# chrished/DEMC.jl

Measured on AMD Instinct MI355X. Metric: chain-updates/sec (N x gens/s) + gens-to-Rhat<1.05, MvNormal d=5 N=1024, higher is better.
Workload: dtype f64

## Files before the change

### demc.jl_amd/csrc/demcz_capi.hip

```cpp
#include "../../include/demcz.h"
#include "demcz_kernels.h"
#include "demcz_kernels_acf.h"
#include "demcz_kernels_sel.h"
#include "demcz_select_host.h"
#include "demcz_kernels_ml.h"
#include "demcz_kernels_pc.h"
#include "demcz_kernels_lr.h"
#include "demcz_kernels_ps.h"
#include "demcz_kernels_ps2.h"
#include "demcz_kernels_ps2d.h"
#include "demcz_pw_dispatch.h"
#include "demcz_mlr_dispatch.h"
#include "demcz_program.h"

#include <rccl/rccl.h>

#include <algorithm>
#include <chrono>
#include <thread>
#include <cstdlib>
#include <deque>
#include <mutex>
#include <cmath>
#include <cstdio>
#include <cstring>
#include <string>
#include <unordered_map>
// ... 192 lines not shown
    bool external_append = false;
    double* dXprop = nullptr;
    double* dlogu = nullptr;
    bool proposal_pending = false;
    bool gen_open = false;
    double* hc_X = nullptr;
    double* hc_lp = nullptr;
    volatile unsigned int* hc_flag = nullptr;
    unsigned int* hc_count = nullptr;
    unsigned int hc_seq = 0;
    hipStream_t diag_stream = nullptr;
    hipEvent_t diag_ev = nullptr;
    hipEvent_t rhat_side_ev = nullptr;
    bool rhat_side_pending = false;
    double* d_spec_X = nullptr;
    double* d_spec_lp = nullptr;
    hipEvent_t spec_ev = nullptr;
    double* pinned_rhat = nullptr;
    unsigned int* pinned_err = nullptr;
    int64_t pinned_err_launches = -1;
    int64_t pinned_cap = 0;
    bool timing = false;
    std::vector<std::pair<hipEvent_t, hipEvent_t>> timed;
    std::vector<double> series_start_ms, series_dur_ms;
    int64_t timed_launches = 0;
    int64_t live_wg_cap = -1;
    SplitKind split_kind = SPLIT_NONE;
    int split_lanes = 0;
    int split_per_wg = 1;
    int32_t* d_slot_role = nullptr;
    double* d_rec[2] = {nullptr, nullptr};
    unsigned int* d_live_err = nullptr;
#ifdef DEMCZ_STAMPS
    unsigned long long* d_stamps = nullptr;
#endif
    bool arena = false, rec_in_arena = false, hist_joint = false;
    int64_t arena_gens = 0;
    double* arena_rec[2] = {nullptr, nullptr};
    double* arena_temp = nullptr;
    int64_t rec_cap = 0;
    int rec_cur = 0;
    bool host_paced = false;
    int wpw = 1;
    bool ps_dual = false;
    bool dual_now = false;
    bool lr_spec = false;
    bool no_live = false;
    bool live_claimed = false;
    unsigned int live_spin_limit = 0;
    int32_t live_fault_polls = 0;
    int64_t live_fault_g = 0;
    bool in_checked = false;
    struct RunCall { int64_t g_from, g_to; double gamma; bool tempered; std::vector<double> temperature; };
    std::vector<RunCall> live_log;
    double* d_safe_X = nullptr;
    double* d_safe_lp = nullptr;
    bool snap_pending = false;
    int64_t safe_M = 0, safe_M_app = 0, safe_g_done = 0;
    bool replaying = false;
    int32_t live_redos = 0;
// ... 260 lines not shown
static int32_t rec_scrub(demcz_handle* h)
{
    rec_invalidate(h);
    if (h->lanes != DEMCZ_LAYOUT_SPLIT || h->rec_cap <= 0 || getenv("DEMCZ_NO_SCRUB")) return DEMCZ_OK;
    for (int b = 0; b < 2; ++b) {
        if (!h->d_rec[b]) continue;
        const size_t per = h->rec_in_arena ? (size_t)(h->cfg.d + 2) : (size_t)((h->split_kind == SPLIT_MLB) ? 2 * h->S : (int64_t)h->cfg.d + 2);
        const size_t nd = (size_t)h->rec_cap * per * (size_t)h->cfg.N + REC_PAD;
        HIPCHK(h, hipMemsetAsync(h->d_rec[b], 0, nd * sizeof(double), h->stream));
    }
    return DEMCZ_OK;
}
static int32_t flush_exchanges(demcz_handle* h);
static void peer_detach(demcz_handle* h);
static void peer_no_dual(demcz_handle* h);
static int32_t peer_setup_ipc(demcz_handle* h);
static bool peer_capable(const demcz_handle* h);
static int32_t check_live_err(demcz_handle* h);
static int32_t live_verify(demcz_handle* h);
static int32_t group_verify(demcz_handle* h);
static int32_t live_failed(demcz_handle* h, bool& failed);
static void live_release(demcz_handle* h);
static int64_t live_span(demcz_handle* h);
static int32_t rec_reserve(demcz_handle* h, int64_t gens);
static int32_t check_hist_range(demcz_handle* h, int64_t g_from, int64_t g_to, const char* who);
static bool ps2_applicable(const demcz_handle* h, const WindowParams& P);

extern "C" int32_t demcz_abi_version(void) { return DEMCZ_ABI_VERSION; }

extern "C" const char* demcz_last_error(const demcz_handle* h)
{
    return h ? h->err.c_str() : g_create_error.c_str();
}

template <class T>
static hipError_t dev_alloc_copy(T** dst, const T* src, size_t n, hipStream_t s, int device)
{
    hipError_t e = dev_malloc(device, (void**)dst, std::max<size_t>(n, 1) * sizeof(T));
    if (e != hipSuccess) return e;
    if (n) e = hipMemcpyAsync(*dst, src, n * sizeof(T), hipMemcpyHostToDevice, s);
    return e;
}

static void free_all(demcz_handle* h)
{
    bool drained = !h->comm_dead;
// ... 263 lines not shown
            h->lanes = L;
        } else if (cfg->lanes_per_chain == 0 && L > 1 && cfg->N * L <= 262144) {
            h->lanes = L;
        }
    }
    if (h->lanes == DEMCZ_LAYOUT_SPLIT && h->split_kind == SPLIT_ML && cfg->target_kind == DEMCZ_TARGET_LINREG_SSE && !getenv("DEMCZ_NO_LR_SPEC")) {
        int cus = 0;
        if (hipDeviceGetAttribute(&cus, hipDeviceAttributeMultiprocessorCount, cfg->device_id) != hipSuccess) cus = 0;
        if ((cfg->N + LR8_CHAINS - 1) / LR8_CHAINS <= (int64_t)cus && lr8s_dynamic_lds<10>(cfg->nobs) <= ML_MAX_DYNAMIC_LDS) {
            h->lr_spec = true;
            h->split_per_wg = LR8_CHAINS;
        }
    }
    h->cfg.block_offsets = nullptr; h->cfg.block_indices = nullptr; h->cfg.eps_scale = nullptr;
    h->cfg.mu = nullptr; h->cfg.W = nullptr; h->cfg.design = nullptr; h->cfg.yobs = nullptr; h->cfg.stream = nullptr;
    if (cfg->target_kind == DEMCZ_TARGET_PROGRAM) h->cfg.nobs = 0;

    const int64_t N = cfg->N;
    const int64_t N_for_arena = cfg->N;
    h->ZS = (d <= 1) ? 2 : (d <= 2) ? 2 : (d <= 4) ? 4 : ((d + 7) / 8) * 8;
    {
        size_t zbytes = (size_t)cfg->Mcap * h->ZS * sizeof(double);
        if (h->lanes == DEMCZ_LAYOUT_SPLIT && h->split_kind == SPLIT_WAVE && d <= 5 && !h->prog_wave && !getenv("DEMCZ_NO_PS2")) {
            const int64_t per_gen = (int64_t)(d + 2) * N_for_arena * (int64_t)sizeof(double);
            int64_t ag = std::max<int64_t>(cfg->K, std::min<int64_t>((int64_t)((h->ps_dual ? 128ll : 64ll) << 20) / per_gen, 1 << 20));
            if (cfg->Gcap > 0) ag = std::min<int64_t>(ag, std::max<int64_t>(cfg->Gcap, 1024));
            ag = std::max<int64_t>(ag, (int64_t)cfg->K * 4);
            const size_t zb = (zbytes + 255) & ~(size_t)255;
            const size_t rb = (((size_t)ag * (size_t)(d + 2) * (size_t)N_for_arena + REC_PAD) * sizeof(double) + 255) & ~(size_t)255;
            const size_t tb = (((size_t)ag + 64) * sizeof(double) + 255) & ~(size_t)255;
            if (zb + 2 * rb + tb < 0xF0000000ull) {
                h->arena = true;
                h->arena_gens = ag;
                CRCHK(g_dev_pool.acquire((void**)&h->dZ, zb + 2 * rb + tb, cfg->device_id));
                h->dZ_bytes = zb + 2 * rb + tb;
                unsigned char* base = reinterpret_cast<unsigned char*>(h->dZ);
                h->arena_rec[0] = reinterpret_cast<double*>(base + zb);
                h->arena_rec[1] = reinterpret_cast<double*>(base + zb + rb);
                h->arena_temp = reinterpret_cast<double*>(base + zb + 2 * rb);
                CRCHK(hipMemsetAsync(base + zb, 0, 2 * rb + tb, h->stream));
            }
        }
        if (!h->arena) { CRCHK(g_dev_pool.acquire((void**)&h->dZ, zbytes, cfg->device_id)); h->dZ_bytes = zbytes; }
        if (h->ps_dual && !h->arena) { h->ps_dual = false; h->split_per_wg = PS_CHAINS; h->live_wg_cap = -1; }
        h->pooled_dev = true;
    }
    CRCHK(dev_malloc(h->cfg.device_id, (void**)&h->d_live_err, 4 * sizeof(unsigned int)));
    CRCHK(hipMemsetAsync(h->d_live_err, 0, 4 * sizeof(unsigned int), h->stream));
    CRCHK(dev_malloc(h->cfg.device_id, (void**)&h->dX, (size_t)N * d * sizeof(double)));
    CRCHK(dev_malloc(h->cfg.device_id, (void**)&h->dlp, (size_t)N * sizeof(double)));
    if (cfg->Gcap > 0) {
        const size_t skew = getenv("DEMCZ_DEBUG_HIST_SKEW") ? ((size_t)atol(getenv("DEMCZ_DEBUG_HIST_SKEW")) & ~(size_t)7) : 0;
        CRCHK(g_dev_pool.acquire((void**)&h->dchain_alloc, (size_t)N * (d + 1) * cfg->Gcap * sizeof(double) + skew, cfg->device_id));
        h->dchain = h->dchain_alloc + skew / sizeof(double);
        h->dlogobj = h->dchain + (size_t)N * d * cfg->Gcap;
        h->hist_joint = true;
// ... 1252 lines not shown
    std::lock_guard<std::mutex> lk(g_live_mutex);
    const int dev = h->cfg.device_id;
    if (dev >= 0 && dev < 64) g_live_used[dev] = std::max<int64_t>(0, g_live_used[dev] - h->live_share);
    h->live_share = 0;
    h->live_claimed = false;
}

static void peer_no_dual(demcz_handle* h)
{
    if (!h->ps_dual) return;
    live_release(h);
    h->ps_dual = false;
    h->dual_now = false;
    h->split_per_wg = PS_CHAINS;
    h->live_wg_cap = -1;
    rec_invalidate(h);
}

static bool peer_capable(const demcz_handle* h)
{
    return h->lanes == DEMCZ_LAYOUT_SPLIT && h->split_kind != SPLIT_PC8 && h->split_kind != SPLIT_NONE;
}

static int64_t live_span(demcz_handle* h)
{
    if (h->lanes != DEMCZ_LAYOUT_SPLIT || (h->comm && h->peer_mode != 2) || h->lag > 0 || h->external_append || h->no_live) return 0;
    if (h->peer_mode != 0 && !peer_capable(h)) return 0;
    if (h->peer_mode == 1 && (!h->group || h->group->failed || h->group->dead)) return 0;
    static const bool disabled = (getenv("DEMCZ_NO_LIVE") != nullptr);
    if (disabled) return 0;
    const int per_wg = h->split_per_wg;
    if ((h->cfg.N + per_wg - 1) / per_wg > live_wg_capacity(h)) return 0;
    if (!live_claim(h)) return 0;
    const int64_t per_gen = rec_fields(h) * h->cfg.N * (int64_t)sizeof(double);
    static const int64_t env_mib = getenv("DEMCZ_REC_MIB") ? atol(getenv("DEMCZ_REC_MIB")) : 0;
    const int64_t mib = env_mib > 0 ? env_mib : (h->arena ? (h->ps_dual ? 128 : 64) : (h->split_kind == SPLIT_MLB) ? 128 : 1024);
    const int64_t span = (int64_t)(mib << 20) / per_gen;
    return std::max<int64_t>(h->cfg.K, std::min<int64_t>(span, 1 << 20));
}

static int32_t stream_history(demcz_handle* h, int64_t g_from, int64_t g_to)
{
    if (!h->hs_on || h->cfg.Gcap <= 0 || g_to < g_from) return DEMCZ_OK;
    const int64_t N = h->cfg.N, s0 = g_from - h->g0 - 1, G = g_to - g_from + 1;
    const int d = h->cfg.d;
    if (s0 < 0 || s0 + G > h->cfg.Gcap) return DEMCZ_OK;
    hipEvent_t ev = h->after_launch_ev;
    if (!ev) {
        if (!h->diag_ev) HIPCHK(h, hipEventCreateWithFlags(&h->diag_ev, hipEventDisableTiming));
        HIPCHK(h, hipEventRecord(h->diag_ev, h->stream));
        h->after_launch_ev = ev = h->diag_ev;
    }
    HIPCHK(h, hipStreamWaitEvent(h->hs_stream, ev, 0));
    HIPCHK(h, hipMemcpyAsync(h->hs_chain + (size_t)N * d * s0, h->dchain + (size_t)N * d * s0, (size_t)N * d * G * sizeof(double), hipMemcpyDeviceToHost, h->hs_stream));
    HIPCHK(h, hipMemcpyAsync(h->hs_logobj + (size_t)N * s0, h->dlogobj + (size_t)N * s0, (size_t)N * G * sizeof(double), hipMemcpyDeviceToHost, h->hs_stream));
    return DEMCZ_OK;
}

extern "C" int32_t demcz_history_stream(demcz_handle* h, int32_t enabled)
// ... 210 lines not shown
        if (h->ps_dual) {
            const int64_t tb0 = next_boundary - g + 1, rest = g_to - g + 1;
            const bool temp_ok = !temperature || temp_in_arena;
            const bool hist_ok = !hist || (double)h->cfg.N * (h->cfg.d + 1) * (double)h->cfg.Gcap * 8.0 < 4293918720.0;
            const bool reg = K % PS2_R == 0 && tb0 % PS2_R == 0 && rest >= PS2_R && temp_ok && hist_ok && h->arena && h->rec_in_arena;
            if (reg) {
                h->dual_now = true;
                if (live_max > 0) live_max = std::max<int64_t>((std::min(live_max, rest) / PS2_R) * PS2_R, PS2_R);
                else w_end = g + ((w_end - g + 1) / PS2_R) * PS2_R - 1;
            } else {
                live_max = 0;
            }
        }
        if (live_max > 0) {
            int64_t n = std::min(live_max, g_to - g + 1);
            const auto& dc = h->rec_desc[h->rec_cur];
            const int64_t rows_v = h->cfg.N * (peer ? shards : 1);
            const int32_t boff = (int32_t)(K - (next_boundary - g + 1));
            const bool ready = dc.valid && dc.g_first == g + h->rng_offset && dc.M == h->M && dc.rows == rows_v && dc.boff == boff;
            if (ready && dc.ngen >= K) {
                if (dc.ngen < n) n = std::max<int64_t>((dc.ngen / K) * K, K);
            } else {
                const int64_t per_gen = rec_fields(h) * h->cfg.N * (int64_t)sizeof(double);
                const int64_t cold = std::max<int64_t>(K, ((int64_t)((h->ps_dual ? 128ll : 64ll) << 20) / per_gen / K) * K);
                n = std::min(n, cold);
            }
            if (h->dual_now) n = std::max<int64_t>((n / PS2_R) * PS2_R, PS2_R);
            w_end = g + n - 1;
        }
        int32_t rc = admit_pending(h, g);
        if (rc) return rc;
        const int64_t nbound = w_end / K - (g - 1) / K;
        P.M = h->M;
        P.M_append = h->M_app;
        P.g_first = g + h->rng_offset;
        P.ngen = (int32_t)(w_end - g + 1);
        P.to_boundary = (int32_t)(next_boundary - g + 1);
        P.slot_first = hist ? (g - h->g0 - 1) : 0;
        P.temperature = temperature ? (temp_in_arena ? h->arena_temp : h->dtemp) + (g - g_from) : nullptr;
        P.do_append = (nbound > 0 && kernel_appends) ? 1 : 0;
        P.snap = nullptr;
        if (nbound > 0 && rccl_exchange && E > 0) {
            if (h->batch_cnt == 0) {
                if (h->buf_xseq[h->batch_buf] > h->xseq_waited) HIPCHK(h, hipStreamWaitEvent(h->stream, h->buf_done[h->batch_buf], 0));
                h->batch_base = h->M_app;
            }
            P.snap = h->d_send[h->batch_buf] + (size_t)h->batch_cnt * h->cfg.N * h->cfg.d;
        }
        if (h->lanes == DEMCZ_LAYOUT_SPLIT) {
            const int64_t ng = w_end + 1;
            const int64_t nb1 = ((ng - 1) / K + 1) * (int64_t)K;
            int64_t nend = nb1;
            if (E > 0 && !h->external_append) nend = ((nend / K + E - 1) / E) * E * (int64_t)K;
            int64_t nM = h->M, nn = nend - ng + 1;
            const int64_t rows_n = h->cfg.N * shards;
            if (live_max > 0) nn = std::min(live_max, (w_end < g_to) ? g_to - w_end : G);
            if (h->external_append) nn = 0;
            else if (E == 0) nM = h->M_app + nbound * rows_n;
            else for (const auto& pe : h->pending) if (pe.visible_from <= ng) nM = pe.M_after;
            const int64_t vis_rows = (E == 0) ? rows_n : 0;
            const int32_t nboff = (int32_t)(K - (nb1 - ng + 1));
            rc = pc_prepare(h, P, vis_rows, ng + h->rng_offset, nn, nM, vis_rows, nboff);
            if (rc) return rc;
        }
        static const bool force_live = getenv("DEMCZ_FORCE_LIVE_KERNEL") != nullptr;
        const bool live = live_max > 0 && (((w_end - 1) / K - (g - 1) / K) > 0 || peer || force_live);
        P.live_err = h->d_live_err;
        P.live_spin_limit = h->live_spin_limit ? (int32_t)h->live_spin_limit : LIVE_SPIN_LIMIT;
        if (h->live_fault_polls > 0 && g >= h->live_fault_g) P.live_spin_limit = h->live_fault_polls;
        if (h->live_fault_polls < 0 && live && g >= h->live_fault_g)
            HIPCHK(h, hipMemsetAsync(h->d_live_err, 0x01, sizeof(unsigned int), h->stream));
        P.acc_out = h->d_acc ? h->d_acc + (size_t)h->acc_next * (size_t)h->acc_waves * 2 : nullptr;
        if (h->ps_dual && P.acc_out)
            HIPCHK(h, hipMemsetAsync(P.acc_out, 0, (size_t)h->acc_waves * 2 * sizeof(unsigned int), h->stream));
        if (live) h->err_clean = false;
        rc = launch_window(h, P, live);
        h->after_launch_ev = nullptr;
        if (rc) return rc;
        if (h->d_acc) {
// ... 11 lines not shown
            } else {
                for (int64_t j = (g - 1) / K + 1; j <= w_end / K; ++j) {
                    const int64_t J = ((j + E - 1) / E) * E;
                    h->M_app += rows;
                    if (h->batch_J != J) {
                        h->pending.push_back({(J + E) * (int64_t)K + 1, h->M_app, nullptr});
                        h->batch_J = J;
                    } else {
                        h->pending.back().M_after = h->M_app;
                    }
                    if (rccl_exchange) {
                        ++h->batch_cnt;
                        if (j == J) { rc = exchange_batch(h); if (rc) return rc; }
                    }
                }
            }
        }
        g = w_end + 1;
    }
    if (timed) {
        HIPCHK(h, hipEventRecord(tev.b, h->stream));
        h->after_launch_ev = tev.b;
        h->timed.emplace_back(tev.a, tev.b);
        tev.a = tev.b = nullptr;
        h->timed_launches += timed_launches;
    }
    if (rccl_exchange && E > 0) {
        int32_t rc = exchange_batch(h);
        if (rc) return rc;
    }
    h->g_done = g_to;
    return DEMCZ_OK;
}

extern "C" int32_t demcz_synchronize(demcz_handle* h)
{
    if (!h) return DEMCZ_ERR_INVALID_ARGUMENT;
    DEADCHK(h);
    HIPCHK(h, hipSetDevice(h->cfg.device_id));
    SYNCCHK(h, h->stream);
    if (h->comm_stream) SYNCCHK(h, h->comm_stream);
    if (h->prod_stream) SYNCCHK(h, h->prod_stream);
    return live_verify(h);
}

static int32_t check_hist_range(demcz_handle* h, int64_t g_from, int64_t g_to, const char* who)
// ... 91 lines not shown
        rc = ensure_scratch(h, 1);
        if (rc) return rc;
        static_assert(sizeof(long long) == sizeof(double), "scratch reuse");
        hipLaunchKernelGGL(sum_counts_kernel, dim3(1), dim3(256), 0, h->stream, (const unsigned int*)h->d_acc, h->acc_waves,
                           (int)h->acc_log[first].slot, last - first + 1, (int)h->acc_slots, skip, (long long*)h->d_scratch);
        HIPCHK(h, hipGetLastError());
        long long v = 0;
        HIPCHK(h, hipMemcpyAsync(&v, h->d_scratch, sizeof(v), hipMemcpyDeviceToHost, h->stream));
        SYNCCHK(h, h->stream);
        *total = (int64_t)v;
        if (from_ballots) *from_ballots = 1;
        return DEMCZ_OK;
    }
    std::vector<int64_t> ch((size_t)(g_to - g_from + 1));
    rc = demcz_get_changed(h, g_from, g_to, ch.data());
    if (rc) return rc;
    int64_t t = 0;
    for (int64_t v : ch) t += v;
    *total = t;
    if (from_ballots) *from_ballots = 0;
    return DEMCZ_OK;
}

struct RhatPlan { int64_t N, w, s0, n, nd, need; int d, nchunk; double *S1, *S2, *mean_j, *s2_j, *sums; };

static int rhat_chunks(int64_t n) { return (int)std::min<int64_t>(std::max<int64_t>(1, n / 32), 32); }
static int64_t rhat_need(int64_t nd, int d, int nchunk) { return 2 * (2 * nchunk * nd) + 2 * (2 * nd) + 4 * d; }

static int32_t rhat_plan(demcz_handle* h, int64_t g_from, int64_t g_to, RhatPlan& r, const char* who = "demcz_rhat")
{
    int32_t rc = check_hist_range(h, g_from, g_to, who);
    if (rc) return rc;
    r.N = h->cfg.N; r.w = g_to - g_from + 1; r.s0 = g_from - h->g0 - 1; r.d = h->cfg.d;
    r.n = r.w / 2;
    if (r.n < 2) return fail(h, DEMCZ_ERR_INVALID_ARGUMENT, std::string(who) + ": window needs at least 4 generations");
    r.nchunk = rhat_chunks(r.n);
    r.nd = r.N * r.d;
    r.need = rhat_need(r.nd, r.d, r.nchunk);
    return DEMCZ_OK;
}

static int32_t rhat_scratch(demcz_handle* h, RhatPlan& r, int64_t extra, bool compute, hipStream_t qs = nullptr)
{
    HIPCHK(h, hipSetDevice(h->cfg.device_id));
    int32_t rc = ensure_scratch(h, r.need + extra);
    if (rc) return rc;
    r.S1 = h->d_scratch;
    r.S2 = r.S1 + 2 * r.nchunk * r.nd;
    r.mean_j = r.S2 + 2 * r.nchunk * r.nd;
    r.s2_j = r.mean_j + 2 * r.nd;
    r.sums = r.s2_j + 2 * r.nd;
    if (compute) {
        const int bs = 256;
        const unsigned gx = (unsigned)((r.nd + bs - 1) / bs);
        if (!qs) qs = h->stream;
        hipLaunchKernelGGL(rhat_moments_kernel, dim3(gx, 2 * r.nchunk), dim3(bs), 0, qs, h->dchain, r.N, r.d, r.s0, r.n, r.nchunk, r.S1, r.S2);
        hipLaunchKernelGGL(rhat_chainstats_kernel, dim3(gx, 2), dim3(bs), 0, qs, h->dchain, r.N, r.d, r.s0, r.n, r.nchunk, r.S1, r.S2, r.mean_j, r.s2_j);
        HIPCHK(h, hipGetLastError());
    }
    return DEMCZ_OK;
}

static int32_t rhat_prepare(demcz_handle* h, int64_t g_from, int64_t g_to, RhatPlan& r, bool compute, hipStream_t qs = nullptr)
{
    int32_t rc = rhat_plan(h, g_from, g_to, r);
    if (rc) return rc;
    return rhat_scratch(h, r, 0, compute, qs);
}

extern "C" int32_t demcz_rhat_partial(demcz_handle* h, int64_t g_from, int64_t g_to, int32_t stage, const double* grand, double* out)
{
    if (!h || !out || (stage != 0 && stage != 1) || (stage == 1 && !grand)) return DEMCZ_ERR_INVALID_ARGUMENT;
    RhatPlan r;
    int32_t rc = live_verify(h);
    if (rc) return rc;
    rc = rhat_prepare(h, g_from, g_to, r, true);
    if (rc) return rc;
    const int d = r.d;
    if (stage == 0) {
        hipLaunchKernelGGL(rhat_reduce_kernel, dim3(d), dim3(256), 0, h->stream, r.mean_j, r.s2_j, r.N, d, 0, (const double*)nullptr, 1.0, r.sums);
        HIPCHK(h, hipGetLastError());
        HIPCHK(h, hipMemcpyAsync(out, r.sums, (size_t)d * sizeof(double), hipMemcpyDeviceToHost, h->stream));
    } else {
        HIPCHK(h, hipMemcpyAsync(r.sums, grand, (size_t)d * sizeof(double), hipMemcpyHostToDevice, h->stream));
        hipLaunchKernelGGL(rhat_reduce_kernel, dim3(d), dim3(256), 0, h->stream, r.mean_j, r.s2_j, r.N, d, 1, (const double*)r.sums, 1.0, r.sums + d);
        HIPCHK(h, hipGetLastError());
        HIPCHK(h, hipMemcpyAsync(out, r.sums + d, (size_t)2 * d * sizeof(double), hipMemcpyDeviceToHost, h->stream));
    }
    SYNCCHK(h, h->stream);
    return DEMCZ_OK;
}

static int32_t rhat_enqueue(demcz_handle* h, int64_t g_from, int64_t g_to, double* out, bool side = false)
{
    RhatPlan r;
    hipStream_t qs = h->stream;
    static const bool own_env = getenv("DEMCZ_RHAT_OWN_STREAM") != nullptr;
    if (side && !h->comm && !own_env && h->prod_stream) {
        if (!h->diag_ev) HIPCHK(h, hipEventCreateWithFlags(&h->diag_ev, hipEventDisableTiming));
        if (h->after_launch_ev) {
            HIPCHK(h, hipStreamWaitEvent(h->prod_stream, h->after_launch_ev, 0));
        } else {
            HIPCHK(h, hipEventRecord(h->diag_ev, h->stream));
            HIPCHK(h, hipStreamWaitEvent(h->prod_stream, h->diag_ev, 0));
            h->after_launch_ev = h->diag_ev;
        }
        qs = h->prod_stream;
    } else if (side && h->comm && h->peer_mode == 2 && !h->no_live && h->comm_side && h->comm_stream && h->lag == 0) {
        if (!h->diag_ev) HIPCHK(h, hipEventCreateWithFlags(&h->diag_ev, hipEventDisableTiming));
        if (h->after_launch_ev) {
            HIPCHK(h, hipStreamWaitEvent(h->comm_stream, h->after_launch_ev, 0));
        } else {
            HIPCHK(h, hipEventRecord(h->diag_ev, h->stream));
            HIPCHK(h, hipStreamWaitEvent(h->comm_stream, h->diag_ev, 0));
            h->after_launch_ev = h->diag_ev;
        }
// ... 2 lines not shown
        if (!h->diag_stream) HIPCHK(h, stream_acquire(h->cfg.device_id, &h->diag_stream));
        if (!h->diag_ev) HIPCHK(h, hipEventCreateWithFlags(&h->diag_ev, hipEventDisableTiming));
        if (h->after_launch_ev) {
            HIPCHK(h, hipStreamWaitEvent(h->diag_stream, h->after_launch_ev, 0));
        } else {
            HIPCHK(h, hipEventRecord(h->diag_ev, h->stream));
            HIPCHK(h, hipStreamWaitEvent(h->diag_stream, h->diag_ev, 0));
            h->after_launch_ev = h->diag_ev;
        }
        qs = h->diag_stream;
    }
    if (qs == h->stream && h->rhat_side_pending) {
        HIPCHK(h, hipStreamWaitEvent(h->stream, h->rhat_side_ev, 0));
        h->rhat_side_pending = false;
    }
    struct SideMark {
        demcz_handle* h; hipStream_t qs;
        ~SideMark() {
            if (qs == h->stream) return;
            if (!h->rhat_side_ev && hipEventCreateWithFlags(&h->rhat_side_ev, hipEventDisableTiming) != hipSuccess) { h->rhat_side_ev = nullptr; return; }
            if (hipEventRecord(h->rhat_side_ev, qs) == hipSuccess) h->rhat_side_pending = true;
        }
    } side_mark{h, qs};
    int32_t rc = rhat_prepare(h, g_from, g_to, r, true, qs);
    if (rc) return rc;
    const int d = r.d;
    const int64_t n = r.n;
    const int64_t m = 2 * r.N * h->nranks;
    const bool sharded = (h->comm != nullptr);
    double* sums = r.sums;
    if (!sharded) {
        hipLaunchKernelGGL(rhat_tail_kernel, dim3(d), dim3(256), 0, qs, r.mean_j, r.s2_j, r.N, d, (double)n, (double)m, sums + 3 * d);
        HIPCHK(h, hipGetLastError());
        HIPCHK(h, hipMemcpyAsync(out, sums + 3 * d, (size_t)d * sizeof(double), hipMemcpyDeviceToHost, qs));
        return DEMCZ_OK;
    }
    const ncclComm_t cq = (qs == h->comm_stream && qs != h->stream) ? h->comm_side : h->comm;
    hipLaunchKernelGGL(rhat_reduce_kernel, dim3(d), dim3(256), 0, qs, r.mean_j, r.s2_j, r.N, d, 0, (const double*)nullptr, 1.0, sums);
    HIPCHK(h, hipGetLastError());
    NCCLCHK(h, ncclAllReduce(sums, sums, (size_t)d, ncclDouble, ncclSum, cq, qs));
    hipLaunchKernelGGL(rhat_reduce_kernel, dim3(d), dim3(256), 0, qs, r.mean_j, r.s2_j, r.N, d, 1, (const double*)sums, (double)m, sums + d);
    HIPCHK(h, hipGetLastError());
    NCCLCHK(h, ncclAllReduce(sums + d, sums + d, (size_t)2 * d, ncclDouble, ncclSum, cq, qs));
    hipLaunchKernelGGL(rhat_final_kernel, dim3((unsigned)((d + 63) / 64)), dim3(64), 0, qs, (const double*)(sums + d), d, (double)n, (double)m, sums + 3 * d);
    HIPCHK(h, hipGetLastError());
    HIPCHK(h, hipMemcpyAsync(out, sums + 3 * d, (size_t)d * sizeof(double), hipMemcpyDeviceToHost, qs));
    return DEMCZ_OK;
}

extern "C" int32_t demcz_rhat(demcz_handle* h, int64_t g_from, int64_t g_to, double* rhat)
{
    if (!h || !rhat) return DEMCZ_ERR_INVALID_ARGUMENT;
    int32_t rc = live_verify(h);
    if (rc) return rc;
    rc = rhat_enqueue(h, g_from, g_to, rhat);
    if (rc) return rc;
    SYNCCHK(h, h->stream);
// ... 1191 lines not shown
        { int32_t rcq = quiesce_all(h); if (rcq) return rcq; }
        SYNCCHK(h, h->stream);
        if (h->pinned_rhat) (void)host_free(h->pinned_rhat);
        h->pinned_rhat = nullptr; h->pinned_cap = 0;
        const int64_t cap = std::max<int64_t>(max_checks, 1024) * d;
        HIPCHK(h, host_malloc((void**)&h->pinned_rhat, (size_t)cap * sizeof(double)));
        h->pinned_cap = cap;
    }
    double* pinned = h->pinned_rhat;
    auto max_of = [d](const double* r) {
        double mx = r[0];
        for (int p = 1; p < d; ++p) mx = (r[p] > mx || r[p] != r[p]) ? r[p] : mx;
        return mx;
    };
    int32_t rc = DEMCZ_OK;
    const bool speculate = !monitor && !h->comm && h->lag == 0 && !h->external_append && !temperature;
    const int64_t N = h->cfg.N;
    if (speculate) {
        if (!h->d_spec_X) HIPCHK(h, dev_malloc(h->cfg.device_id, (void**)&h->d_spec_X, (size_t)N * d * sizeof(double)));
        if (!h->d_spec_lp) HIPCHK(h, dev_malloc(h->cfg.device_id, (void**)&h->d_spec_lp, (size_t)N * sizeof(double)));
        if (!h->spec_ev) HIPCHK(h, hipEventCreateWithFlags(&h->spec_ev, hipEventDisableTiming));
    }
    bool ahead = false;
    while (g <= g_to && rc == DEMCZ_OK) {
        const int64_t nxt = std::min(g_to, ((g - 1) / every + 1) * every);
        if (!ahead) rc = demcz_run(h, g, nxt, gamma, temperature ? temperature + (g - g_from) : nullptr);
        ahead = false;
        if (rc) break;
        if (nxt % every == 0 && nxt - every >= h->g0) {
            double* slot = pinned + (size_t)checks * d;
            rc = rhat_enqueue(h, nxt - every + 1, nxt, slot, monitor && nxt < g_to);
            if (rc) break;
            ++checks;
            if (!monitor) {
                int64_t M_before = 0;
                if (speculate && nxt < g_to) {
                    if (hipEventRecord(h->spec_ev, h->stream) != hipSuccess) { rc = fail(h, DEMCZ_ERR_HIP, "demcz_run_checked: event failed"); break; }
                    if (hipMemcpyAsync(h->d_spec_X, h->dX, (size_t)N * d * sizeof(double), hipMemcpyDeviceToDevice, h->stream) != hipSuccess ||
                        hipMemcpyAsync(h->d_spec_lp, h->dlp, (size_t)N * sizeof(double), hipMemcpyDeviceToDevice, h->stream) != hipSuccess) {
                        rc = fail(h, DEMCZ_ERR_HIP, "demcz_run_checked: snapshot failed");
                        break;
                    }
                    M_before = h->M_app;
                    const int64_t nn = std::min(g_to, (nxt / every + 1) * every);
                    rc = demcz_run(h, nxt + 1, nn, gamma, nullptr);
                    if (rc) break;
                    ahead = true;
                    if ((rc = sync_event(h, h->spec_ev, "demcz_run_checked")) != DEMCZ_OK) break;
                } else if ((rc = sync_stream(h, h->stream, "demcz_run_checked")) != DEMCZ_OK) {
                    break;
                }
                if (max_of(slot) < threshold) {
                    if (g_stop) *g_stop = nxt;
                    if (ahead) {
                        if ((rc = sync_stream(h, h->stream, "demcz_run_checked")) != DEMCZ_OK) break;
                        rc = check_live_err(h);
// ... 202 lines not shown
    rec_invalidate(h);
    return DEMCZ_OK;
}

extern "C" int32_t demcz_set_kernel_timing(demcz_handle* h, int32_t enabled)
{
    if (!h) return DEMCZ_ERR_INVALID_ARGUMENT;
    h->timing = enabled != 0;
    return DEMCZ_OK;
}

extern "C" int32_t demcz_get_kernel_time(demcz_handle* h, int64_t* launches, double* milliseconds)
{
    if (!h) return DEMCZ_ERR_INVALID_ARGUMENT;
    HIPCHK(h, hipSetDevice(h->cfg.device_id));
    SYNCCHK(h, h->stream);
    double total = 0.0;
    h->after_launch_ev = nullptr;
    h->series_start_ms.clear(); h->series_dur_ms.clear();
    for (auto& pr : h->timed) {
        float ms = 0.0f, st = 0.0f;
        HIPCHK(h, hipEventElapsedTime(&ms, pr.first, pr.second));
        if (&pr != &h->timed.front()) HIPCHK(h, hipEventElapsedTime(&st, h->timed.front().first, pr.first));
        h->series_start_ms.push_back(st); h->series_dur_ms.push_back(ms);
        total += ms;
    }
    for (auto& pr : h->timed) {
        (void)hipEventDestroy(pr.first);
        (void)hipEventDestroy(pr.second);
    }
    if (launches) *launches = h->timed_launches;
    if (milliseconds) *milliseconds = total;
    h->timed.clear();
    h->timed_launches = 0;
    return DEMCZ_OK;
}

extern "C" int32_t demcz_get_kernel_time_series(demcz_handle* h, int32_t cap, double* start_ms, double* duration_ms, int32_t* n)
{
    if (!h || cap < 0 || !n) return DEMCZ_ERR_INVALID_ARGUMENT;
    const int32_t m = (int32_t)std::min<size_t>(h->series_start_ms.size(), (size_t)cap);
    for (int32_t i = 0; i < m; ++i) {
        if (start_ms) start_ms[i] = h->series_start_ms[i];
        if (duration_ms) duration_ms[i] = h->series_dur_ms[i];
    }
    *n = (int32_t)h->series_start_ms.size();
    return DEMCZ_OK;
}
```

### demc.jl_amd/csrc/demcz_kernels.h

```cpp
#pragma once

#include "demcz_device.h"

#pragma clang fp contract(off)

#ifdef DEMCZ_STAMPS
#define DEMCZ_STAMP(P, i) do { if ((P).stamps && threadIdx.x == 0 && blockIdx.x < 65536u) (P).stamps[(size_t)blockIdx.x * 16 + (i)] = __builtin_readcyclecounter(); } while (0)
#else
#define DEMCZ_STAMP(P, i) do { } while (0)
#endif

namespace demcz {

enum { TARGET_MVNORMAL = 0, TARGET_ISO_QUAD = 1, TARGET_LINREG_SSE = 2, TARGET_HOST_CALLBACK = 3, TARGET_PROGRAM = 4 };

constexpr int MAX_D = 64;
constexpr int LINREG_PARTIALS = 16;
constexpr int WINDOW_BS = 64;

struct TargetParams {
    const double* mu;
    const double* Wp;
    double c0;
    const double* design;
// ... 507 lines not shown
    out[r + ldout * p] = Z[(r0 + r) * ZS + p];
}

__global__ void append_gathered_kernel(double* Z, int64_t ZS, int64_t M, const double* slab, int64_t n_loc,
                                       int R, int d)
{
    const int64_t i = (int64_t)blockIdx.x * blockDim.x + threadIdx.x;
    const int64_t per = n_loc * d;
    if (i >= per * R) return;
    const int64_t r = i / per, rem = i % per, p = rem / n_loc, j = rem % n_loc;
    Z[(M + r * n_loc + j) * ZS + p] = slab[i];
}

__global__ void append_batch_kernel(double* Z, int64_t ZS, int64_t base, const double* slab, int64_t n_loc, int R, int cnt, int d)
{
    const int64_t i = (int64_t)blockIdx.x * blockDim.x + threadIdx.x;
    const int64_t per = n_loc * d;
    if (i >= per * cnt * R) return;
    const int64_t r = i / (per * cnt), rem = i % (per * cnt), sidx = rem / per, rem2 = rem % per, p = rem2 / n_loc, j = rem2 % n_loc;
    Z[(base + (sidx * R + r) * n_loc + j) * ZS + p] = slab[i];
}

__global__ void rhat_moments_kernel(const double* chain, int64_t N, int d, int64_t s0, int64_t n, int nchunk,
                                    double* S1, double* S2)
{
    const int64_t i = (int64_t)blockIdx.x * blockDim.x + threadIdx.x;
    if (i >= N * d) return;
    const int h = blockIdx.y / nchunk, ck = blockIdx.y % nchunk;
    const int64_t per = (n + nchunk - 1) / nchunk;
    const int64_t t0 = ck * per, t1 = (t0 + per < n) ? t0 + per : n;
    const int64_t stride = N * d;
    const double* base = chain + i + stride * (s0 + h * n);
    const double x0 = base[0];
    double a = 0.0, b = 0.0;
    int64_t t = t0;
    for (; t + 8 <= t1; t += 8) {
        double v[8];
#pragma unroll
        for (int u = 0; u < 8; ++u) v[u] = base[stride * (t + u)];
#pragma unroll
        for (int u = 0; u < 8; ++u) {
            const double w = v[u] - x0;
            a += w;
            b = fma(w, w, b);
        }
    }
    for (; t < t1; ++t) {
        double v = base[stride * t] - x0;
        a += v;
        b = fma(v, v, b);
    }
    const int64_t o = i + stride * blockIdx.y;
    S1[o] = a;
    S2[o] = b;
}

__global__ void rhat_chainstats_kernel(const double* chain, int64_t N, int d, int64_t s0, int64_t n, int nchunk,
                                       const double* S1, const double* S2, double* mean_j, double* s2_j)
{
    const int64_t i = (int64_t)blockIdx.x * blockDim.x + threadIdx.x;
    if (i >= N * d) return;
    const int h = blockIdx.y;
    const int64_t stride = N * d;
    const double x0 = chain[i + stride * (s0 + h * n)];
    double a = 0.0, b = 0.0;
    for (int ck = 0; ck < nchunk; ++ck) {
        a += S1[i + stride * (h * nchunk + ck)];
        b += S2[i + stride * (h * nchunk + ck)];
    }
    const double nn = (double)n;
    mean_j[i + stride * h] = x0 + a / nn;
    s2_j[i + stride * h] = (b - a * a / nn) / (nn - 1.0);
}

__global__ void __launch_bounds__(256) rhat_reduce_kernel(const double* mean_j, const double* s2_j, int64_t N, int d,
                                                          int stage, const double* grand, double grand_div, double* out)
{
    __shared__ double ra[256], rb[256];
    const int p = blockIdx.x;
    const int64_t stride = N * d;
    double a = 0.0, b = 0.0;
    const double gm = stage ? grand[p] / grand_div : 0.0;
    int64_t h = 0, c = threadIdx.x;
    while (c >= N) { c -= N; ++h; }
// ... 7 lines not shown
            a = fma(dv, dv, a);
            b += s2_j[at];
        }
        c += 256;
        while (c >= N) { c -= N; ++h; }
    }
    ra[threadIdx.x] = a;
    rb[threadIdx.x] = b;
    __syncthreads();
    for (int s = 128; s > 0; s >>= 1) {
        if ((int)threadIdx.x < s) {
            ra[threadIdx.x] += ra[threadIdx.x + s];
            rb[threadIdx.x] += rb[threadIdx.x + s];
        }
        __syncthreads();
    }
    if (threadIdx.x == 0) {
        out[p] = ra[0];
        if (stage) out[d + p] = rb[0];
    }
}

__global__ void __launch_bounds__(256) rhat_tail_kernel(const double* mean_j, const double* s2_j, int64_t N, int d,
                                                        double n, double m, double* rhat)
{
    __shared__ double ra[256], rb[256];
    const int p = blockIdx.x;
    const int64_t stride = N * d;
    double a = 0.0, b = 0.0;
    int64_t h0 = 0, c0 = threadIdx.x;
    while (c0 >= N) { c0 -= N; ++h0; }
    {
        int64_t h = h0, c = c0;
        for (int64_t k = threadIdx.x; k < 2 * N; k += 256) {
            a += mean_j[c + N * p + stride * h];
            c += 256;
            while (c >= N) { c -= N; ++h; }
        }
    }
    ra[threadIdx.x] = a;
    __syncthreads();
    for (int s = 128; s > 0; s >>= 1) {
        if ((int)threadIdx.x < s) ra[threadIdx.x] += ra[threadIdx.x + s];
        __syncthreads();
    }
    const double gm = ra[0] / m;
    __syncthreads();
    a = 0.0;
    {
        int64_t h = h0, c = c0;
// ... 185 lines not shown
```

Baseline: 682.6 million.

## Batch monitored runs across multiple check slabs with batched Rhat kernels

In monitored, unsharded runs the sampler now advances several convergence-check intervals in one run call instead of stopping at every check boundary. The per-interval Rhat statistics for all covered intervals are then computed together by launching the moments, chainstats and tail kernels with an extra grid dimension over slabs, followed by a single copy back to host. This is meant to cut per-interval launch, synchronisation and host round-trip overhead. Arena sizing moves into a helper that can shrink the span to fit the size limit, and timing brackets are split evenly across slabs. The trade-off is more scratch memory and Rhat values that arrive later, which can delay stopping once convergence is reached.

Result: faster. 722.1 million, median of 6 (+5.8%).

```diff
diff --git a/demc.jl_amd/csrc/demcz_capi.hip b/demc.jl_amd/csrc/demcz_capi.hip
--- a/demc.jl_amd/csrc/demcz_capi.hip
+++ b/demc.jl_amd/csrc/demcz_capi.hip
@@ -3,6 +3,7 @@
 #include "demcz_kernels_acf.h"
 #include "demcz_kernels_sel.h"
 #include "demcz_select_host.h"
+#include "demcz_slab_plan.h"
 #include "demcz_kernels_ml.h"
 #include "demcz_kernels_pc.h"
 #include "demcz_kernels_lr.h"
@@ -241,6 +242,9 @@
     int64_t pinned_cap = 0;
     bool timing = false;
     std::vector<std::pair<hipEvent_t, hipEvent_t>> timed;
+    std::vector<int32_t> timed_slabs;
+    int32_t bracket_slabs = 1;
+    int64_t plan_next = 0;
     std::vector<double> series_start_ms, series_dur_ms;
     int64_t timed_launches = 0;
     int64_t live_wg_cap = -1;
@@ -255,6 +259,7 @@
 #endif
     bool arena = false, rec_in_arena = false, hist_joint = false;
     int64_t arena_gens = 0;
+    int64_t arena_span = 0;
     double* arena_rec[2] = {nullptr, nullptr};
     double* arena_temp = nullptr;
     int64_t rec_cap = 0;
@@ -561,6 +566,7 @@
 static int32_t live_failed(demcz_handle* h, bool& failed);
 static void live_release(demcz_handle* h);
 static int64_t live_span(demcz_handle* h);
+static int64_t rec_target_bytes(bool dual);
 static int32_t rec_reserve(demcz_handle* h, int64_t gens);
 static int32_t check_hist_range(demcz_handle* h, int64_t g_from, int64_t g_to, const char* who);
 static bool ps2_applicable(const demcz_handle* h, const WindowParams& P);
@@ -870,16 +876,13 @@
     {
         size_t zbytes = (size_t)cfg->Mcap * h->ZS * sizeof(double);
         if (h->lanes == DEMCZ_LAYOUT_SPLIT && h->split_kind == SPLIT_WAVE && d <= 5 && !h->prog_wave && !getenv("DEMCZ_NO_PS2")) {
-            const int64_t per_gen = (int64_t)(d + 2) * N_for_arena * (int64_t)sizeof(double);
-            int64_t ag = std::max<int64_t>(cfg->K, std::min<int64_t>((int64_t)((h->ps_dual ? 128ll : 64ll) << 20) / per_gen, 1 << 20));
-            if (cfg->Gcap > 0) ag = std::min<int64_t>(ag, std::max<int64_t>(cfg->Gcap, 1024));
-            ag = std::max<int64_t>(ag, (int64_t)cfg->K * 4);
-            const size_t zb = (zbytes + 255) & ~(size_t)255;
-            const size_t rb = (((size_t)ag * (size_t)(d + 2) * (size_t)N_for_arena + REC_PAD) * sizeof(double) + 255) & ~(size_t)255;
-            const size_t tb = (((size_t)ag + 64) * sizeof(double) + 255) & ~(size_t)255;
-            if (zb + 2 * rb + tb < 0xF0000000ull) {
+            const ArenaSpan as = arena_span(zbytes, N_for_arena, d, cfg->K, cfg->Gcap, rec_target_bytes(h->ps_dual), (int64_t)REC_PAD);
+            const int64_t ag = as.gens;
+            const size_t zb = as.zb, rb = as.rb, tb = as.tb;
+            if (ag > 0 && zb + 2 * rb + tb < ARENA_LIMIT) {
                 h->arena = true;
                 h->arena_gens = ag;
+                h->arena_span = as.span;
                 CRCHK(g_dev_pool.acquire((void**)&h->dZ, zb + 2 * rb + tb, cfg->device_id));
                 h->dZ_bytes = zb + 2 * rb + tb;
                 unsigned char* base = reinterpret_cast<unsigned char*>(h->dZ);
@@ -2178,6 +2181,18 @@
     return h->lanes == DEMCZ_LAYOUT_SPLIT && h->split_kind != SPLIT_PC8 && h->split_kind != SPLIT_NONE;
 }
 
+static int64_t rec_env_mib()
+{
+    static const int64_t env_mib = getenv("DEMCZ_REC_MIB") ? atol(getenv("DEMCZ_REC_MIB")) : 0;
+    return env_mib;
+}
+
+static int64_t rec_target_bytes(bool dual)
+{
+    const int64_t mib = rec_env_mib() > 0 ? rec_env_mib() : (dual ? 2 * ARENA_REC_MIB : ARENA_REC_MIB);
+    return mib << 20;
+}
+
 static int64_t live_span(demcz_handle* h)
 {
     if (h->lanes != DEMCZ_LAYOUT_SPLIT || (h->comm && h->peer_mode != 2) || h->lag > 0 || h->external_append || h->no_live) return 0;
@@ -2189,8 +2204,9 @@
     if ((h->cfg.N + per_wg - 1) / per_wg > live_wg_capacity(h)) return 0;
     if (!live_claim(h)) return 0;
     const int64_t per_gen = rec_fields(h) * h->cfg.N * (int64_t)sizeof(double);
-    static const int64_t env_mib = getenv("DEMCZ_REC_MIB") ? atol(getenv("DEMCZ_REC_MIB")) : 0;
-    const int64_t mib = env_mib > 0 ? env_mib : (h->arena ? (h->ps_dual ? 128 : 64) : (h->split_kind == SPLIT_MLB) ? 128 : 1024);
+    if (h->arena) return std::max<int64_t>(h->cfg.K, std::min<int64_t>(h->arena_span, SPAN_GENS_MAX));
+    const int64_t env_mib = rec_env_mib();
+    const int64_t mib = env_mib > 0 ? env_mib : (h->split_kind == SPLIT_MLB) ? 128 : 1024;
     const int64_t span = (int64_t)(mib << 20) / per_gen;
     return std::max<int64_t>(h->cfg.K, std::min<int64_t>(span, 1 << 20));
 }
@@ -2447,7 +2463,7 @@
                 if (dc.ngen < n) n = std::max<int64_t>((dc.ngen / K) * K, K);
             } else {
                 const int64_t per_gen = rec_fields(h) * h->cfg.N * (int64_t)sizeof(double);
-                const int64_t cold = std::max<int64_t>(K, ((int64_t)((h->ps_dual ? 128ll : 64ll) << 20) / per_gen / K) * K);
+                const int64_t cold = std::max<int64_t>(K, ((int64_t)((h->ps_dual ? 2 * COLD_REC_MIB : COLD_REC_MIB) << 20) / per_gen / K) * K);
                 n = std::min(n, cold);
             }
             if (h->dual_now) n = std::max<int64_t>((n / PS2_R) * PS2_R, PS2_R);
@@ -2479,7 +2495,7 @@
             if (E > 0 && !h->external_append) nend = ((nend / K + E - 1) / E) * E * (int64_t)K;
             int64_t nM = h->M, nn = nend - ng + 1;
             const int64_t rows_n = h->cfg.N * shards;
-            if (live_max > 0) nn = std::min(live_max, (w_end < g_to) ? g_to - w_end : G);
+            if (live_max > 0) nn = std::min(live_max, (w_end < g_to) ? g_to - w_end : (h->plan_next > 0 ? h->plan_next : G));
             if (h->external_append) nn = 0;
             else if (E == 0) nM = h->M_app + nbound * rows_n;
             else for (const auto& pe : h->pending) if (pe.visible_from <= ng) nM = pe.M_after;
@@ -2537,6 +2553,7 @@
         HIPCHK(h, hipEventRecord(tev.b, h->stream));
         h->after_launch_ev = tev.b;
         h->timed.emplace_back(tev.a, tev.b);
+        h->timed_slabs.push_back(std::max(h->bracket_slabs, 1));
         tev.a = tev.b = nullptr;
         h->timed_launches += timed_launches;
     }
@@ -2674,7 +2691,7 @@
     return DEMCZ_OK;
 }
 
-struct RhatPlan { int64_t N, w, s0, n, nd, need; int d, nchunk; double *S1, *S2, *mean_j, *s2_j, *sums; };
+struct RhatPlan { int64_t N, w, s0, n, nd, need; int d, nchunk; double *S1, *S2, *mean_j, *s2_j, *sums; int slabs = 1; double* out = nullptr; };
 
 static int rhat_chunks(int64_t n) { return (int)std::min<int64_t>(std::max<int64_t>(1, n / 32), 32); }
 static int64_t rhat_need(int64_t nd, int d, int nchunk) { return 2 * (2 * nchunk * nd) + 2 * (2 * nd) + 4 * d; }
@@ -2695,28 +2712,36 @@
 static int32_t rhat_scratch(demcz_handle* h, RhatPlan& r, int64_t extra, bool compute, hipStream_t qs = nullptr)
 {
     HIPCHK(h, hipSetDevice(h->cfg.device_id));
-    int32_t rc = ensure_scratch(h, r.need + extra);
+    int32_t rc = ensure_scratch(h, r.need * r.slabs + (r.slabs > 1 ? (int64_t)r.slabs * r.d : 0) + extra);
     if (rc) return rc;
     r.S1 = h->d_scratch;
     r.S2 = r.S1 + 2 * r.nchunk * r.nd;
     r.mean_j = r.S2 + 2 * r.nchunk * r.nd;
     r.s2_j = r.mean_j + 2 * r.nd;
     r.sums = r.s2_j + 2 * r.nd;
+    r.out = r.slabs > 1 ? h->d_scratch + r.need * r.slabs : r.sums + 3 * r.d;
     if (compute) {
         const int bs = 256;
         const unsigned gx = (unsigned)((r.nd + bs - 1) / bs);
         if (!qs) qs = h->stream;
-        hipLaunchKernelGGL(rhat_moments_kernel, dim3(gx, 2 * r.nchunk), dim3(bs), 0, qs, h->dchain, r.N, r.d, r.s0, r.n, r.nchunk, r.S1, r.S2);
-        hipLaunchKernelGGL(rhat_chainstats_kernel, dim3(gx, 2), dim3(bs), 0, qs, h->dchain, r.N, r.d, r.s0, r.n, r.nchunk, r.S1, r.S2, r.mean_j, r.s2_j);
+        hipLaunchKernelGGL(rhat_moments_kernel, dim3(gx, 2 * r.nchunk, r.slabs), dim3(bs), 0, qs, h->dchain, r.N, r.d, r.s0, r.n, r.nchunk, r.S1, r.S2,
+                           r.w, r.need);
+        hipLaunchKernelGGL(rhat_chainstats_kernel, dim3(gx, 2, r.slabs), dim3(bs), 0, qs, h->dchain, r.N, r.d, r.s0, r.n, r.nchunk, r.S1, r.S2, r.mean_j,
+                           r.s2_j, r.w, r.need);
         HIPCHK(h, hipGetLastError());
     }
     return DEMCZ_OK;
 }
 
-static int32_t rhat_prepare(demcz_handle* h, int64_t g_from, int64_t g_to, RhatPlan& r, bool compute, hipStream_t qs = nullptr)
+static int32_t rhat_prepare(demcz_handle* h, int64_t g_from, int64_t g_to, RhatPlan& r, bool compute, hipStream_t qs = nullptr, int slabs = 1)
 {
     int32_t rc = rhat_plan(h, g_from, g_to, r);
     if (rc) return rc;
+    if (slabs > 1) {
+        rc = check_hist_range(h, g_from, g_from + r.w * slabs - 1, "demcz_run_checked");
+        if (rc) return rc;
+        r.slabs = slabs;
+    }
     return rhat_scratch(h, r, 0, compute, qs);
 }
 
@@ -2743,7 +2768,7 @@
     return DEMCZ_OK;
 }
 
-static int32_t rhat_enqueue(demcz_handle* h, int64_t g_from, int64_t g_to, double* out, bool side = false)
+static int32_t rhat_enqueue(demcz_handle* h, int64_t g_from, int64_t g_to, double* out, bool side = false, int slabs = 1)
 {
     RhatPlan r;
     hipStream_t qs = h->stream;
@@ -2792,7 +2817,8 @@
             if (hipEventRecord(h->rhat_side_ev, qs) == hipSuccess) h->rhat_side_pending = true;
         }
     } side_mark{h, qs};
-    int32_t rc = rhat_prepare(h, g_from, g_to, r, true, qs);
+    if (slabs > 1 && h->comm) return fail(h, DEMCZ_ERR_STATE, "demcz_run_checked: batched checks are for unsharded runs");
+    int32_t rc = rhat_prepare(h, g_from, g_to, r, true, qs, slabs);
     if (rc) return rc;
     const int d = r.d;
     const int64_t n = r.n;
@@ -2800,9 +2826,9 @@
     const bool sharded = (h->comm != nullptr);
     double* sums = r.sums;
     if (!sharded) {
-        hipLaunchKernelGGL(rhat_tail_kernel, dim3(d), dim3(256), 0, qs, r.mean_j, r.s2_j, r.N, d, (double)n, (double)m, sums + 3 * d);
+        hipLaunchKernelGGL(rhat_tail_kernel, dim3(d, r.slabs), dim3(256), 0, qs, r.mean_j, r.s2_j, r.N, d, (double)n, (double)m, r.out, r.need);
         HIPCHK(h, hipGetLastError());
-        HIPCHK(h, hipMemcpyAsync(out, sums + 3 * d, (size_t)d * sizeof(double), hipMemcpyDeviceToHost, qs));
+        HIPCHK(h, hipMemcpyAsync(out, r.out, (size_t)r.slabs * d * sizeof(double), hipMemcpyDeviceToHost, qs));
         return DEMCZ_OK;
     }
     const ncclComm_t cq = (qs == h->comm_stream && qs != h->stream) ? h->comm_side : h->comm;
@@ -4040,16 +4066,42 @@
         if (!h->spec_ev) HIPCHK(h, hipEventCreateWithFlags(&h->spec_ev, hipEventDisableTiming));
     }
     bool ahead = false;
+    const bool grouped = monitor && !h->comm && h->lag == 0 && !h->external_append;
+    int64_t max_slabs = 1;
+    if (grouped && h->cfg.Gcap > 0) {
+        const int64_t need1 = rhat_need(N * d, d, rhat_chunks(every / 2));
+        const int64_t ls0 = live_span(h);
+        max_slabs = std::max<int64_t>(1, std::min<int64_t>(std::min<int64_t>(SLAB_GROUP_MAX, ((int64_t)1 << 25) / need1), (ls0 > 0 ? ls0 : h->cfg.Gcap) / every + 1));
+        rc = ensure_scratch(h, max_slabs * (need1 + d));
+    }
+    auto cut_now = [h]() {
+        int64_t cut = 0;
+        if (h->live_fault_polls != 0) cut = h->live_fault_g;
+        if (h->no_live && h->rearm_from >= 0 && (cut == 0 || h->rearm_from + 1 < cut)) cut = h->rearm_from + 1;
+        return cut;
+    };
     while (g <= g_to && rc == DEMCZ_OK) {
-        const int64_t nxt = std::min(g_to, ((g - 1) / every + 1) * every);
+        int64_t nxt = std::min(g_to, ((g - 1) / every + 1) * every);
+        if (grouped) {
+            const int64_t ls = live_span(h);
+            const int64_t span = ls > 0 ? ls : INT64_MAX;
+            nxt = slab_group_end(g, g_to, every, span, cut_now(), max_slabs);
+            h->bracket_slabs = (int32_t)(slab_ends_in(g, nxt, every) + (nxt % every != 0 ? 1 : 0));
+            h->plan_next = nxt < g_to ? std::min<int64_t>(span, slab_group_end(nxt + 1, g_to, every, span, cut_now(), max_slabs) - nxt) : 0;
+        }
         if (!ahead) rc = demcz_run(h, g, nxt, gamma, temperature ? temperature + (g - g_from) : nullptr);
+        h->bracket_slabs = 1;
+        h->plan_next = 0;
         ahead = false;
         if (rc) break;
-        if (nxt % every == 0 && nxt - every >= h->g0) {
+        int64_t c0 = slab_end_at_or_after(g, every);
+        while (c0 <= nxt && c0 - every < h->g0) c0 += every;
+        const int64_t nck = c0 <= nxt ? (nxt - c0) / every + 1 : 0;
+        if (nck > 0) {
             double* slot = pinned + (size_t)checks * d;
-            rc = rhat_enqueue(h, nxt - every + 1, nxt, slot, monitor && nxt < g_to);
+            rc = rhat_enqueue(h, c0 - every + 1, c0, slot, monitor && nxt < g_to, (int)nck);
             if (rc) break;
-            ++checks;
+            checks += (int32_t)nck;
             if (!monitor) {
                 int64_t M_before = 0;
                 if (speculate && nxt < g_to) {
@@ -4298,7 +4350,8 @@
         float ms = 0.0f, st = 0.0f;
         HIPCHK(h, hipEventElapsedTime(&ms, pr.first, pr.second));
         if (&pr != &h->timed.front()) HIPCHK(h, hipEventElapsedTime(&st, h->timed.front().first, pr.first));
-        h->series_start_ms.push_back(st); h->series_dur_ms.push_back(ms);
+        const int32_t k = h->timed_slabs[(size_t)(&pr - &h->timed.front())];
+        for (int32_t i = 0; i < k; ++i) { h->series_start_ms.push_back((double)st + i * ((double)ms / k)); h->series_dur_ms.push_back((double)ms / k); }
         total += ms;
     }
     for (auto& pr : h->timed) {
@@ -4308,6 +4361,7 @@
     if (launches) *launches = h->timed_launches;
     if (milliseconds) *milliseconds = total;
     h->timed.clear();
+    h->timed_slabs.clear();
     h->timed_launches = 0;
     return DEMCZ_OK;
 }
diff --git a/demc.jl_amd/csrc/demcz_kernels.h b/demc.jl_amd/csrc/demcz_kernels.h
--- a/demc.jl_amd/csrc/demcz_kernels.h
+++ b/demc.jl_amd/csrc/demcz_kernels.h
@@ -553,10 +553,13 @@
 }
 
 __global__ void rhat_moments_kernel(const double* chain, int64_t N, int d, int64_t s0, int64_t n, int nchunk,
-                                    double* S1, double* S2)
+                                    double* S1, double* S2, int64_t w, int64_t slice)
 {
     const int64_t i = (int64_t)blockIdx.x * blockDim.x + threadIdx.x;
     if (i >= N * d) return;
+    s0 += (int64_t)blockIdx.z * w;
+    S1 += (int64_t)blockIdx.z * slice;
+    S2 += (int64_t)blockIdx.z * slice;
     const int h = blockIdx.y / nchunk, ck = blockIdx.y % nchunk;
     const int64_t per = (n + nchunk - 1) / nchunk;
     const int64_t t0 = ck * per, t1 = (t0 + per < n) ? t0 + per : n;
@@ -587,10 +590,15 @@
 }
 
 __global__ void rhat_chainstats_kernel(const double* chain, int64_t N, int d, int64_t s0, int64_t n, int nchunk,
-                                       const double* S1, const double* S2, double* mean_j, double* s2_j)
+                                       const double* S1, const double* S2, double* mean_j, double* s2_j, int64_t w, int64_t slice)
 {
     const int64_t i = (int64_t)blockIdx.x * blockDim.x + threadIdx.x;
     if (i >= N * d) return;
+    s0 += (int64_t)blockIdx.z * w;
+    S1 += (int64_t)blockIdx.z * slice;
+    S2 += (int64_t)blockIdx.z * slice;
+    mean_j += (int64_t)blockIdx.z * slice;
+    s2_j += (int64_t)blockIdx.z * slice;
     const int h = blockIdx.y;
     const int64_t stride = N * d;
     const double x0 = chain[i + stride * (s0 + h * n)];
@@ -644,10 +652,13 @@
 }
 
 __global__ void __launch_bounds__(256) rhat_tail_kernel(const double* mean_j, const double* s2_j, int64_t N, int d,
-                                                        double n, double m, double* rhat)
+                                                        double n, double m, double* rhat, int64_t slice)
 {
     __shared__ double ra[256], rb[256];
     const int p = blockIdx.x;
+    mean_j += (int64_t)blockIdx.y * slice;
+    s2_j += (int64_t)blockIdx.y * slice;
+    rhat += (int64_t)blockIdx.y * d;
     const int64_t stride = N * d;
     double a = 0.0, b = 0.0;
     int64_t h0 = 0, c0 = threadIdx.x;
diff --git a/demc.jl_amd/csrc/demcz_slab_plan.h b/demc.jl_amd/csrc/demcz_slab_plan.h
--- /dev/null
+++ b/demc.jl_amd/csrc/demcz_slab_plan.h
@@ -0,0 +1,93 @@
+#pragma once
+
+#include <cstdint>
+
+namespace demcz {
+
+constexpr uint64_t ARENA_LIMIT = 0xF0000000ull;
+constexpr int64_t SPAN_GENS_MAX = (int64_t)1 << 20;
+constexpr int64_t ARENA_REC_MIB = 64;
+constexpr int64_t COLD_REC_MIB = 64;
+
+struct ArenaSpan {
+    int64_t gens;
+    int64_t span;
+    uint64_t zb, rb, tb;
+};
+
+inline uint64_t arena_total(const ArenaSpan& a) { return a.zb + 2 * a.rb + a.tb; }
+
+inline void arena_sizes(ArenaSpan& a, uint64_t zbytes, int64_t N, int d, int64_t rec_pad)
+{
+    a.zb = (zbytes + 255) & ~(uint64_t)255;
+    a.rb = (((uint64_t)a.gens * (uint64_t)(d + 2) * (uint64_t)N + (uint64_t)rec_pad) * 8 + 255) & ~(uint64_t)255;
+    a.tb = (((uint64_t)a.gens + 64) * 8 + 255) & ~(uint64_t)255;
+}
+
+inline ArenaSpan arena_span(uint64_t zbytes, int64_t N, int d, int64_t K, int64_t Gcap, int64_t target_bytes, int64_t rec_pad)
+{
+    ArenaSpan a{0, 0, 0, 0, 0};
+    const int64_t per_gen = (int64_t)(d + 2) * N * 8;
+    int64_t span = target_bytes / per_gen;
+    if (span > SPAN_GENS_MAX) span = SPAN_GENS_MAX;
+    if (span < K) span = K;
+    auto gens_of = [&](int64_t s) {
+        int64_t g = s;
+        if (Gcap > 0 && g > (Gcap > 1024 ? Gcap : 1024)) g = (Gcap > 1024 ? Gcap : 1024);
+        if (g < 4 * K) g = 4 * K;
+        return g;
+    };
+    a.gens = gens_of(span);
+    arena_sizes(a, zbytes, N, d, rec_pad);
+    if (arena_total(a) >= ARENA_LIMIT) {
+        const uint64_t fixed = ((zbytes + 255) & ~(uint64_t)255) + 2 * ((uint64_t)rec_pad * 8 + 256) + (64 * 8 + 256);
+        if (fixed >= ARENA_LIMIT) return ArenaSpan{0, 0, 0, 0, 0};
+        int64_t fit = (int64_t)((ARENA_LIMIT - fixed) / (2 * (uint64_t)per_gen + 8));
+        if (fit > span) fit = span;
+        for (;; --fit) {
+            if (fit < 4 * K || fit < 1) return ArenaSpan{0, 0, 0, 0, 0};
+            a.gens = fit;
+            arena_sizes(a, zbytes, N, d, rec_pad);
+            if (arena_total(a) < ARENA_LIMIT) break;
+        }
+        for (; fit < span; ++fit) {
+            a.gens = fit + 1;
+            arena_sizes(a, zbytes, N, d, rec_pad);
+            if (arena_total(a) >= ARENA_LIMIT) break;
+        }
+        span = fit;
+        a.gens = gens_of(span);
+        arena_sizes(a, zbytes, N, d, rec_pad);
+    }
+    a.span = span;
+    return a;
+}
+
+constexpr int SLAB_TAIL_GROUP_MAX = 1;
+constexpr int SLAB_GROUP_MAX = 64;
+
+inline int64_t slab_end_at_or_after(int64_t g, int64_t every) { return ((g + every - 1) / every) * every; }
+
+inline int64_t slab_group_end(int64_t g, int64_t g_to, int64_t every, int64_t span, int64_t cut, int64_t max_slabs = SLAB_GROUP_MAX)
+{
+    const int64_t e1 = slab_end_at_or_after(g, every);
+    if (e1 >= g_to) return g_to;
+    const int64_t last_start = ((g_to - 1) / every) * every + 1;
+    const int64_t lim = last_start - 1;
+    int64_t e = lim;
+    if (span < e - g + 1) e = ((g + span - 1) / every) * every;
+    if (max_slabs < 1) max_slabs = 1;
+    if (max_slabs > SLAB_GROUP_MAX) max_slabs = SLAB_GROUP_MAX;
+    if ((e - e1) / every + 1 > max_slabs) e = e1 + (max_slabs - 1) * every;
+    if (cut > g) {
+        const int64_t ec = slab_end_at_or_after(cut - 1, every);
+        if (e > ec) e = ec;
+    }
+    if (e < e1) e = e1;
+    if (e == lim && (e - e1) / every + 1 > SLAB_TAIL_GROUP_MAX) e = lim - (int64_t)SLAB_TAIL_GROUP_MAX * every;
+    return e;
+}
+
+inline int64_t slab_ends_in(int64_t g, int64_t e, int64_t every) { return e / every - (g - 1) / every; }
+
+}
```
